# voidful/DeSTA2.5-Audio

Measured on AMD Instinct MI355X. Metric: train steps/sec (node) Whisper-v3+Llama3.1-8B Q-Former6L at 1/2/4/8 MI355X, higher is better.
Workload: dtype bf16

## Files before the change

desta2.5-audio_amd/csrc/gemm_bf16.hip:

```cpp
#include "common.h"
#include "desta_hip.h"
#include <math.h>

#ifndef GEMM_GROUP_M
#define GEMM_GROUP_M 8
#endif

namespace {

typedef __attribute__((ext_vector_type(4))) unsigned u32x4;
typedef __attribute__((ext_vector_type(2))) float f32x2;

constexpr int BM = 128, BN = 128, BK = 64;
constexpr int TILE_BYTES = BM * BK * 2;

struct GemmArgs {
    const bf16_t* A; const bf16_t* B; void* C;
    int M, N, K;
    long lda, ldb, ldc;
    long sA, sB, sC;
    const float* bias;
    const void* res; long ldr; long sR; int res_f32;
    int act;
    int out_f32;
// ... 381 lines not shown
        bf16x4_t v;
        asm volatile("ds_read_b64_tr_b16 %0, %1" : "=v"(v) : "v"((unsigned)(unsigned long)(img + off)) : "memory");
        o[4 * s2 + 0] = v[0]; o[4 * s2 + 1] = v[1]; o[4 * s2 + 2] = v[2]; o[4 * s2 + 3] = v[3];
    }
    return o;
}

template <bool TA, bool TB>
__global__ __launch_bounds__(256, 2) void gemm_bf16_nt_ring_kernel(GemmArgs p) {
    constexpr int NS = 4;
    __shared__ __attribute__((aligned(16))) char lds[NS * 2 * TILE_BYTES];

    const int tid = threadIdx.x, lane = tid & 63, wave = __builtin_amdgcn_readfirstlane(tid >> 6);
    const int wr = wave >> 1, wc = wave & 1;

    const int ntile = p.tilesM * p.tilesN;
    const int L = xcd_remap(blockIdx.x, ntile);
    constexpr int GROUP_M = 8;
    const int gspan = GROUP_M * p.tilesN;
    const int first_m = (L / gspan) * GROUP_M;
    const int gsz = min(p.tilesM - first_m, GROUP_M);
    const int tm = first_m + (L % gspan) % gsz;
    const int tn = (L % gspan) / gsz;
    const int brow = tm * BM, bcol = tn * BN;
    const int z = blockIdx.y;

    const bf16_t* A = p.A + (long)z * p.sA;
    const bf16_t* B = p.B + (long)z * p.sB;

    const bf16_t* srcA[4];
    const bf16_t* srcB[4];
#pragma unroll
    for (int i = 0; i < 4; ++i) {
        const int idx = i * 256 + tid;
        if (TA) {
            const int k = idx >> 4, c = (idx & 15) ^ tr_swz(k);
            srcA[i] = A + (long)k * p.lda + min(brow + c * 8, p.M - 8);
        } else {
            const int r = idx >> 3, c = (idx & 7) ^ (r & 7);
            srcA[i] = A + (long)min(brow + r, p.M - 1) * p.lda + c * 8;
        }
        if (TB) {
            const int k = idx >> 4, c = (idx & 15) ^ tr_swz(k);
            srcB[i] = B + (long)k * p.ldb + min(bcol + c * 8, p.N - 8);
        } else {
            const int r = idx >> 3, c = (idx & 7) ^ (r & 7);
            srcB[i] = B + (long)min(bcol + r, p.N - 1) * p.ldb + c * 8;
        }
    }
    const long stepA = TA ? (long)BK * p.lda : BK, stepB = TB ? (long)BK * p.ldb : BK;
    const int nk = p.K / BK;
    auto stage = [&](int kt) {
        const int kc = min(kt, nk - 1);
        char* la = lds + (kt & (NS - 1)) * 2 * TILE_BYTES;
        char* lb = la + TILE_BYTES;
#pragma unroll
        for (int i = 0; i < 4; ++i) {
            const int wbase = (i * 256 + wave * 64) * 16;
            glds16(srcA[i] + kc * stepA, la + wbase);
            glds16(srcB[i] + kc * stepB, lb + wbase);
        }
    };

    f32x4 acc[4][4];
#pragma unroll
    for (int i = 0; i < 4; ++i)
#pragma unroll
        for (int j = 0; j < 4; ++j) acc[i][j] = f32x4{0.f, 0.f, 0.f, 0.f};

    const int fr = lane & 15, fq = lane >> 4;
    int offA[4], offB[4];
#pragma unroll
    for (int i = 0; i < 4; ++i) {
        const int ra = wr * 64 + i * 16 + fr;
        const int rb = wc * 64 + i * 16 + fr;
        offA[i] = ra * 128 + ((fq ^ (ra & 7)) << 4);
        offB[i] = rb * 128 + ((fq ^ (rb & 7)) << 4);
    }
    auto rd_a = [&](int kt, int kk, int i) __attribute__((always_inline)) -> bf16x8 {
        const char* la = lds + (kt & (NS - 1)) * 2 * TILE_BYTES;
        if (TA) return frag_trans_raw(la, wr * 64 + i * 16, kk, fr, fq);
        return *(const bf16x8*)(la + (offA[i] ^ (kk << 6)));
    };
    auto rd_b = [&](int kt, int kk, int i) __attribute__((always_inline)) -> bf16x8 {
        const char* lb = lds + (kt & (NS - 1)) * 2 * TILE_BYTES + TILE_BYTES;
        if (TB) return frag_trans_raw(lb, wc * 64 + i * 16, kk, fr, fq);
        return *(const bf16x8*)(lb + (offB[i] ^ (kk << 6)));
    };
    auto fence = [&]() __attribute__((always_inline)) { if (TA || TB) __builtin_amdgcn_sched_barrier(0); };
    auto landed = [&](bf16x8 (&af)[4], bf16x8 (&bfr)[4]) __attribute__((always_inline)) {
        asm volatile("s_waitcnt lgkmcnt(0)" : "+v"(af[0]), "+v"(af[1]), "+v"(af[2]), "+v"(af[3]), "+v"(bfr[0]), "+v"(bfr[1]), "+v"(bfr[2]), "+v"(bfr[3]) :: "memory");
    };

    stage(0); stage(1); stage(2);
    asm volatile("s_waitcnt vmcnt(16)" ::: "memory");
    __builtin_amdgcn_s_barrier();
    bf16x8 a0[4], b0[4], a1[4], b1[4];
#pragma unroll
    for (int i = 0; i < 4; ++i) { a0[i] = rd_a(0, 0, i); b0[i] = rd_b(0, 0, i); }
    landed(a0, b0);
    for (int kt = 0; kt < nk; ++kt) {
        {
            const int kc = min(kt + 3, nk - 1);
            char* la = lds + ((kt + 3) & (NS - 1)) * 2 * TILE_BYTES;
            char* lb = la + TILE_BYTES;
#pragma unroll
            for (int i = 0; i < 4; ++i) {
                const int wbase = (i * 256 + wave * 64) * 16;
                acc[i][0] = __builtin_amdgcn_mfma_f32_16x16x32_bf16(b0[0], a0[i], acc[i][0], 0, 0, 0);
                glds16(srcA[i] + kc * stepA, la + wbase);
                fence();
                acc[i][1] = __builtin_amdgcn_mfma_f32_16x16x32_bf16(b0[1], a0[i], acc[i][1], 0, 0, 0);
                a1[i] = rd_a(kt, 1, i);
                fence();
                acc[i][2] = __builtin_amdgcn_mfma_f32_16x16x32_bf16(b0[2], a0[i], acc[i][2], 0, 0, 0);
                glds16(srcB[i] + kc * stepB, lb + wbase);
                fence();
                acc[i][3] = __builtin_amdgcn_mfma_f32_16x16x32_bf16(b0[3], a0[i], acc[i][3], 0, 0, 0);
                b1[i] = rd_b(kt, 1, i);
                fence();
            }
            if (!TA && !TB) {
#pragma unroll
                for (int i = 0; i < 8; ++i) {
                    __builtin_amdgcn_sched_group_barrier(0x008, 1, 0);
                    __builtin_amdgcn_sched_group_barrier(0x020, 1, 0);
                    __builtin_amdgcn_sched_group_barrier(0x008, 1, 0);
                    __builtin_amdgcn_sched_group_barrier(0x100, 1, 0);
                }
            }
        }
        __builtin_amdgcn_sched_barrier(0);
        landed(a1, b1);
        asm volatile("s_waitcnt vmcnt(16)" ::: "memory");
        __builtin_amdgcn_s_barrier();
#pragma unroll
        for (int i = 0; i < 4; ++i) {
            acc[i][0] = __builtin_amdgcn_mfma_f32_16x16x32_bf16(b1[0], a1[i], acc[i][0], 0, 0, 0);
            acc[i][1] = __builtin_amdgcn_mfma_f32_16x16x32_bf16(b1[1], a1[i], acc[i][1], 0, 0, 0);
            a0[i] = rd_a(kt + 1, 0, i);
            fence();
            acc[i][2] = __builtin_amdgcn_mfma_f32_16x16x32_bf16(b1[2], a1[i], acc[i][2], 0, 0, 0);
            acc[i][3] = __builtin_amdgcn_mfma_f32_16x16x32_bf16(b1[3], a1[i], acc[i][3], 0, 0, 0);
            b0[i] = rd_b(kt + 1, 0, i);
            fence();
        }
        if (!TA && !TB) {
#pragma unroll
            for (int i = 0; i < 8; ++i) {
                __builtin_amdgcn_sched_group_barrier(0x008, 2, 0);
                __builtin_amdgcn_sched_group_barrier(0x100, 1, 0);
            }
        }
        __builtin_amdgcn_sched_barrier(0);
        landed(a0, b0);
    }
    asm volatile("s_waitcnt vmcnt(0)" ::: "memory");

    if constexpr (!TA && !TB) {
        if (p.act == 2 || p.act == 3) {
            const int ncol0 = bcol + wc * 64;
            if (ncol0 < p.N) {
#pragma unroll
                for (int i = 0; i < 4; ++i) {
                    const int m = brow + wr * 64 + i * 16 + fr;
                    if (p.act == 2) epilogue_swiglu_fwd(p, z, min(m, p.M - 1), m < p.M, ncol0, fq, acc[i][0], acc[i][1], acc[i][2], acc[i][3]);
                    else epilogue_swiglu_bwd(p, z, min(m, p.M - 1), m < p.M, ncol0, fq, acc[i][0], acc[i][1], acc[i][2], acc[i][3]);
                }
            }
            return;
        }
    }
#pragma unroll
    for (int i = 0; i < 4; ++i) {
        const int m = brow + wr * 64 + i * 16 + fr;
        if (m >= p.M) continue;
#pragma unroll
        for (int j = 0; j < 4; ++j) {
            const int n0 = bcol + wc * 64 + j * 16 + fq * 4;
            if (n0 >= p.N) continue;
            epilogue4<true>(p, z, m, n0, acc[i][j]);
        }
    }
}


constexpr int HT = 128 * BK * 2;

struct K256Stream {
    const bf16_t* src[4][2];
    char* lds;
    int kt0, nk, n_ht, wave;
    bool tskip;
    __device__ __forceinline__ void init(const GemmArgs& p, char* lds_, int tid, int wave_, const bf16_t* A, const bf16_t* B,
                                         int brow, int bcol, int kt0_, int nk_, bool tskip_) {
        lds = lds_; wave = wave_; kt0 = kt0_; nk = nk_; n_ht = 4 * nk_; tskip = tskip_;
#pragma unroll
        for (int i = 0; i < 2; ++i) {
            const int idx = i * 512 + tid;
            const int r = idx >> 3, pc = idx & 7;
            const int c = pc ^ (r & 7);
#pragma unroll
            for (int s2 = 0; s2 < 2; ++s2) {
                const int arow = (r >> 6) * 128 + s2 * 64 + (r & 63);
                const int bcolr = (r >> 5) * 64 + s2 * 32 + (r & 31);
                src[s2][i] = A + (long)min(brow + arow, p.M - 1) * p.lda + c * 8;
                src[2 + s2][i] = B + (long)min(bcol + bcolr, p.N - 1) * p.ldb + c * 8;
            }
        }
    }
    __device__ __forceinline__ void stage(int j) {
        if (tskip && j >= n_ht) return;
        const int t = j >> 2, q = j & 3;
        const int kind = (q == 0) ? 0 : (q == 1) ? 2 : (q == 2) ? 3 : 1;
        const long koff = (long)(kt0 + min(t, nk - 1)) * BK;
        char* dst = lds + ((t & 1) * 4 + kind) * HT;
#pragma unroll
        for (int i = 0; i < 2; ++i)
            glds16(src[kind][i] + koff, dst + (i * 512 + wave * 64) * 16);
    }
    __device__ __forceinline__ void stage_steady(int j) {
        const int t = j >> 2, q = j & 3;
        const int kind = (q == 0) ? 0 : (q == 1) ? 2 : (q == 2) ? 3 : 1;
        const long koff = (long)(kt0 + t) * BK;
        char* dst = lds + ((t & 1) * 4 + kind) * HT;
#pragma unroll
        for (int i = 0; i < 2; ++i)
            glds16(src[kind][i] + koff, dst + (i * 512 + wave * 64) * 16);
    }
    __device__ __forceinline__ void wait_steady(int) { asm volatile("s_waitcnt vmcnt(8)" ::: "memory"); }
    __device__ __forceinline__ void tail_wait(int issued) {
        const int ov = tskip ? issued - n_ht : 0;
        if (ov <= 0) asm volatile("s_waitcnt vmcnt(8)" ::: "memory");
        else if (ov == 1) asm volatile("s_waitcnt vmcnt(6)" ::: "memory");
        else if (ov == 2) asm volatile("s_waitcnt vmcnt(4)" ::: "memory");
        else if (ov == 3) asm volatile("s_waitcnt vmcnt(2)" ::: "memory");
        else asm volatile("s_waitcnt vmcnt(0)" ::: "memory");
    }
};

template <bool STAGGER, class AtTail>
__device__ __forceinline__ void k256_loop_2phase(K256Stream& st, const int (&offA)[4], const int (&offB)[2], f32x4 (&acc)[8][4],
                                                 AtTail&& at_tail) {
    const int nk = st.nk, wave = st.wave;
    const char* lds = st.lds;
    bf16x8 a[4][2], b0[2][2], b1[2][2];
#define MFMA_SLOT(ACC_I0, ACC_J0, BF)                                                                        \
    __builtin_amdgcn_sched_barrier(0);                                                                       \
    __builtin_amdgcn_s_setprio(1);                                                                           \
    _Pragma("unroll") for (int kk = 0; kk < 2; ++kk)                                                         \
        _Pragma("unroll") for (int i = 0; i < 4; ++i)                                                        \
            _Pragma("unroll") for (int j = 0; j < 2; ++j)                                                    \
                acc[ACC_I0 + i][ACC_J0 + j] =                                                                \
                    __builtin_amdgcn_mfma_f32_16x16x32_bf16(BF[j][kk], a[i][kk], acc[ACC_I0 + i][ACC_J0 + j], 0, 0, 0); \
    __builtin_amdgcn_s_setprio(0);                                                                           \
    __builtin_amdgcn_sched_barrier(0);
#define KTILE_2PHASE(STAGE, WAIT)                                                                              \
    {                                                                                                          \
        _Pragma("unroll") for (int i = 0; i < 2; ++i)                                                          \
            _Pragma("unroll") for (int kk = 0; kk < 2; ++kk) {                                                 \
                b0[i][kk] = *(const bf16x8*)(B0 + (offB[i] ^ (kk << 6)));                                      \
                b1[i][kk] = *(const bf16x8*)(B1 + (offB[i] ^ (kk << 6)));                                      \
            }                                                                                                  \
        _Pragma("unroll") for (int i = 0; i < 4; ++i)                                                          \
            _Pragma("unroll") for (int kk = 0; kk < 2; ++kk) a[i][kk] = *(const bf16x8*)(A0 + (offA[i] ^ (kk << 6))); \
        st.STAGE(g + 7);                                                                                       \
        asm volatile("s_waitcnt lgkmcnt(0)" ::: "memory");                                                     \
        if (STAGGER) { st.WAIT(g + 8); __builtin_amdgcn_s_barrier(); }                                         \
        MFMA_SLOT(0, 0, b0)                                                                                    \
        MFMA_SLOT(0, 2, b1)                                                                                    \
        st.WAIT(g + 8); __builtin_amdgcn_s_barrier();                                                          \
        _Pragma("unroll") for (int i = 0; i < 4; ++i)                                                          \
            _Pragma("unroll") for (int kk = 0; kk < 2; ++kk) a[i][kk] = *(const bf16x8*)(A1 + (offA[i] ^ (kk << 6))); \
        st.STAGE(g + 8);                                                                                       \
        st.STAGE(g + 9);                                                                                       \
        st.STAGE(g + 10);                                                                                      \
        asm volatile("s_waitcnt lgkmcnt(0)" ::: "memory");                                                     \
        if (STAGGER) { st.WAIT(g + 11); __builtin_amdgcn_s_barrier(); }                                       \
        MFMA_SLOT(4, 2, b1)                                                                                    \
        MFMA_SLOT(4, 0, b0)                                                                                    \
        st.WAIT(g + 11); __builtin_amdgcn_s_barrier();                                                         \
    }
    if (STAGGER && wave >= 4) __builtin_amdgcn_s_barrier();
    const int nk_steady = max(nk - 2, 0);
    for (int t = 0; t < nk_steady; ++t) {
        const char* base = lds + (t & 1) * 4 * HT;
        const char* A0 = base, *A1 = base + HT, *B0 = base + 2 * HT, *B1 = base + 3 * HT;
        const int g = 4 * t;
        KTILE_2PHASE(stage_steady, wait_steady)
    }
    at_tail();
    for (int t = nk_steady; t < nk; ++t) {
        const char* base = lds + (t & 1) * 4 * HT;
        const char* A0 = base, *A1 = base + HT, *B0 = base + 2 * HT, *B1 = base + 3 * HT;
        const int g = 4 * t;
        KTILE_2PHASE(stage, tail_wait)
    }
    if (STAGGER && wave < 4) __builtin_amdgcn_s_barrier();
#undef KTILE_2PHASE
#undef MFMA_SLOT
}

constexpr int E256_DYN = -2, E256_SWIGLU_FWD = 32, E256_SWIGLU_BWD = 33, E256_F32_STREAM = 64;
template <int EPI>
__device__ __forceinline__ void k256_epilogue(const GemmArgs& p, int z, int brow, int bcol, int wm, int wn, int fr, int fq,
                                              const f32x4 (&acc)[8][4]) {
    if constexpr (EPI == E256_SWIGLU_FWD || EPI == E256_SWIGLU_BWD) {
        const int ncol0 = bcol + wn * 64;
        if (ncol0 < p.N) {
#pragma unroll
            for (int i = 0; i < 8; ++i) {
                const int m = brow + wm * 128 + i * 16 + fr;
                if (EPI == E256_SWIGLU_FWD) epilogue_swiglu_fwd(p, z, min(m, p.M - 1), m < p.M, ncol0, fq, acc[i][0], acc[i][1], acc[i][2], acc[i][3]);
                else epilogue_swiglu_bwd(p, z, min(m, p.M - 1), m < p.M, ncol0, fq, acc[i][0], acc[i][1], acc[i][2], acc[i][3]);
            }
        }
        return;
    }
#define DESTA_WIDE_TILE(MODE)                                                                                          \
        _Pragma("unroll") for (int i = 0; i < 8; ++i) {                                                                \
            const int m = brow + wm * 128 + i * 16 + fr;                                                               \
            const int mc = min(m, p.M - 1);                                                                            \
            _Pragma("unroll") for (int j = 0; j < 4; j += 2) {                                                         \
                const int ncol0 = bcol + wn * 64 + j * 16;                                                             \
                if (ncol0 >= p.N) continue;                                                          \
                epilogue_pair_bf16<MODE>(p, z, mc, m < p.M, ncol0, fq, acc[i][j], acc[i][j + 1]);    \
            }                                                                                                          \
        }
#define DESTA_F32_STREAM_TILE()                                                                                        \
        _Pragma("unroll") for (int i = 0; i < 8; ++i) {                                                                \
            const int m = brow + wm * 128 + i * 16 + fr;                                                               \
            if (m >= p.M) continue;                                                                                    \
            _Pragma("unroll") for (int j = 0; j < 4; ++j) {                                                            \
                const int n0 = bcol + wn * 64 + j * 16 + fq * 4;                                                       \
                if (n0 >= p.N) continue;                                                                               \
                epilogue4_f32_stream(p, z, m, n0, acc[i][j]);                                                          \
            }                                                                                                          \
        }
    if constexpr (EPI == E256_F32_STREAM) {
        DESTA_F32_STREAM_TILE()
    } else if constexpr (EPI >= 0) {
        DESTA_WIDE_TILE(EPI)
    } else {
        const bool pre_ok = !p.preact || (p.act == 0 && !p.res && (p.ldp & 7) == 0 && (p.sP & 7) == 0);
        const bool wide = !p.out_f32 && pre_ok && p.act <= 1 && !p.drop_thresh && (p.N % 32 == 0) && (p.ldc % 8 == 0);
        if (wide) {
            DESTA_WIDE_TILE(-1)
            return;
        }
#pragma unroll
        for (int i = 0; i < 8; ++i) {
            const int m = brow + wm * 128 + i * 16 + fr;
            if (m >= p.M) continue;
#pragma unroll
            for (int j = 0; j < 4; ++j) {
                const int n0 = bcol + wn * 64 + j * 16 + fq * 4;
                if (n0 >= p.N) continue;
                epilogue4(p, z, m, n0, acc[i][j]);
            }
        }
    }
#undef DESTA_F32_STREAM_TILE
#undef DESTA_WIDE_TILE
}

__device__ __forceinline__ void k256_store_slab(float* slab, int wm, int wn, int fr, int fq, const f32x4 (&acc)[8][4]) {
#pragma unroll
    for (int i = 0; i < 8; ++i)
#pragma unroll
        for (int j = 0; j < 4; ++j)
            *(f32x4*)(slab + (wm * 128 + i * 16 + fr) * 256 + wn * 64 + j * 16 + fq * 4) = acc[i][j];
}

template <bool STAGGER, int PHASES, int EPI = 0>
__global__ __launch_bounds__(512, 2) void gemm_bf16_nt_256_kernel(GemmArgs p) {
    __shared__ __attribute__((aligned(16))) char lds[2 * 4 * HT];

    const int tid = threadIdx.x, lane = tid & 63, wave = __builtin_amdgcn_readfirstlane(tid >> 6);
    const int wm = wave >> 2, wn = wave & 3;

    int L, slice = 0;
    if ((int)blockIdx.x < p.full_tiles) {
        L = xcd_remap(blockIdx.x, p.full_tiles);
    } else {
        const int j = blockIdx.x - p.full_tiles;
        L = p.full_tiles + j / p.split;
        slice = j % p.split;
    }
    constexpr int GROUP_M = GEMM_GROUP_M;
    const int gspan = GROUP_M * p.tilesN;
    const int first_m = (L / gspan) * GROUP_M;
    const int gsz = min(p.tilesM - first_m, GROUP_M);
    const int tm = first_m + (L % gspan) % gsz;
    const int tn = (L % gspan) / gsz;
    const int brow = tm * 256, bcol = tn * 256;
    const int z = blockIdx.y;
    const bf16_t* A = p.A + (long)z * p.sA;
    const bf16_t* B = p.B + (long)z * p.sB;

    const int nk_all = p.K / BK;
    const bool partial = (int)blockIdx.x >= p.full_tiles && p.split > 1;
    const int kt0 = partial ? (int)((long)nk_all * slice / p.split) : 0;
    const int kt1 = partial ? (int)((long)nk_all * (slice + 1) / p.split) : nk_all;
    const int nk = kt1 - kt0;
    K256Stream st;
    st.init(p, lds, tid, wave, A, B, brow, bcol, kt0, nk, PHASES == 2 && p.tail_skip != 0);

    f32x4 acc[8][4];
#pragma unroll
    for (int i = 0; i < 8; ++i)
#pragma unroll
        for (int j = 0; j < 4; ++j) acc[i][j] = f32x4{0.f, 0.f, 0.f, 0.f};

    const int fr = lane & 15, fq = lane >> 4;
    int offA[4], offB[2];
#pragma unroll
    for (int i = 0; i < 4; ++i) {
        const int r = wm * 64 + i * 16 + fr;
        offA[i] = r * 128 + ((fq ^ (r & 7)) << 4);
    }
#pragma unroll
    for (int i = 0; i < 2; ++i) {
        const int r = wn * 32 + i * 16 + fr;
        offB[i] = r * 128 + ((fq ^ (r & 7)) << 4);
    }

#pragma unroll
    for (int j = 0; j < 7; ++j) st.stage(j);
    if (PHASES == 4) asm volatile("s_waitcnt vmcnt(10)" ::: "memory");
    else st.tail_wait(7);
    __builtin_amdgcn_s_barrier();

    if constexpr (PHASES == 2) {
        k256_loop_2phase<STAGGER>(st, offA, offB, acc, [] {});
    } else {
        bf16x8 a[4][2], b0[2][2], b1[2][2];
#define SLOT_END()                                                                                                  \
    asm volatile("s_waitcnt vmcnt(10)" ::: "memory");                                                               \
    __builtin_amdgcn_s_barrier();
#define MFMA_SLOT(ACC_I0, ACC_J0, BF)                                                                        \
    __builtin_amdgcn_sched_barrier(0);                                                                       \
    __builtin_amdgcn_s_setprio(1);                                                                           \
    _Pragma("unroll") for (int kk = 0; kk < 2; ++kk)                                                         \
        _Pragma("unroll") for (int i = 0; i < 4; ++i)                                                        \
            _Pragma("unroll") for (int j = 0; j < 2; ++j)                                                    \
                acc[ACC_I0 + i][ACC_J0 + j] =                                                                \
                    __builtin_amdgcn_mfma_f32_16x16x32_bf16(BF[j][kk], a[i][kk], acc[ACC_I0 + i][ACC_J0 + j], 0, 0, 0); \
    __builtin_amdgcn_s_setprio(0);                                                                           \
    __builtin_amdgcn_sched_barrier(0);
        if (STAGGER && wave >= 4) __builtin_amdgcn_s_barrier();
        for (int t = 0; t < nk; ++t) {
            const char* base = lds + (t & 1) * 4 * HT;
            const char* A0 = base, *A1 = base + HT, *B0 = base + 2 * HT, *B1 = base + 3 * HT;
            const int g = 4 * t;
#pragma unroll
            for (int i = 0; i < 2; ++i)
#pragma unroll
                for (int kk = 0; kk < 2; ++kk) b0[i][kk] = *(const bf16x8*)(B0 + (offB[i] ^ (kk << 6)));
#pragma unroll
            for (int i = 0; i < 4; ++i)
#pragma unroll
                for (int kk = 0; kk < 2; ++kk) a[i][kk] = *(const bf16x8*)(A0 + (offA[i] ^ (kk << 6)));
            st.stage(g + 7);
            asm volatile("s_waitcnt lgkmcnt(0)" ::: "memory");
            if (STAGGER) { SLOT_END() }
            MFMA_SLOT(0, 0, b0)
            SLOT_END()
#pragma unroll
            for (int i = 0; i < 2; ++i)
#pragma unroll
                for (int kk = 0; kk < 2; ++kk) b1[i][kk] = *(const bf16x8*)(B1 + (offB[i] ^ (kk << 6)));
            st.stage(g + 8);
            asm volatile("s_waitcnt lgkmcnt(0)" ::: "memory");
            if (STAGGER) { SLOT_END() }
            MFMA_SLOT(0, 2, b1)
            SLOT_END()
#pragma unroll
            for (int i = 0; i < 4; ++i)
#pragma unroll
                for (int kk = 0; kk < 2; ++kk) a[i][kk] = *(const bf16x8*)(A1 + (offA[i] ^ (kk << 6)));
            st.stage(g + 9);
            asm volatile("s_waitcnt lgkmcnt(0)" ::: "memory");
            if (STAGGER) { SLOT_END() }
            MFMA_SLOT(4, 2, b1)
            SLOT_END()
            st.stage(g + 10);
            if (STAGGER) { SLOT_END() }
            MFMA_SLOT(4, 0, b0)
            SLOT_END()
        }
        if (STAGGER && wave < 4) __builtin_amdgcn_s_barrier();
#undef MFMA_SLOT
#undef SLOT_END
    }
    asm volatile("s_waitcnt vmcnt(0)" ::: "memory");

    if (partial) {
        float* slab = p.ws + ((long)z * (p.tilesM * p.tilesN - p.full_tiles) * p.split +
                              (long)(blockIdx.x - p.full_tiles)) * (256 * 256);
        k256_store_slab(slab, wm, wn, fr, fq, acc);
        if (!p.tickets) return;
        __shared__ int s_go;
        int* tk = p.tickets + 2 * ((long)z * (p.tilesM * p.tilesN - p.full_tiles) + (L - p.full_tiles));
        asm volatile("s_waitcnt vmcnt(0)" ::: "memory");
        __syncthreads();
        if (tid == 0) {
            __builtin_amdgcn_fence(__ATOMIC_RELEASE, "agent");
            asm volatile("s_waitcnt vmcnt(0)" ::: "memory");
            __hip_atomic_fetch_add(tk, 1, __ATOMIC_RELAXED, __HIP_MEMORY_SCOPE_AGENT);
            int spins = 0, ok = 1;
            while (__hip_atomic_load(tk, __ATOMIC_RELAXED, __HIP_MEMORY_SCOPE_AGENT) < p.split) {
                __builtin_amdgcn_s_sleep(2);
                if (++spins > (1 << 21)) { ok = 0; break; }
            }
            __builtin_amdgcn_fence(__ATOMIC_ACQUIRE, "agent");
            asm volatile("s_waitcnt vmcnt(0)" ::: "memory");
            s_go = ok;
        }
        __syncthreads();
        if (s_go) {
            const float* s0 = p.ws + ((long)z * (p.tilesM * p.tilesN - p.full_tiles) + (L - p.full_tiles)) * p.split * (256 * 256);
            const int r0 = 256 * slice / p.split, r1 = 256 * (slice + 1) / p.split;
            for (int idx = tid; idx < (r1 - r0) * 64; idx += 512) {
                const int ml = r0 + (idx >> 6), nl = (idx & 63) * 4;
                const float* q = s0 + ml * 256 + nl;
                f32x4 v = *(const f32x4*)q;
                for (int s2 = 1; s2 < p.split; ++s2) {
                    const f32x4 w = *(const f32x4*)(q + (long)s2 * (256 * 256));
                    v[0] += w[0]; v[1] += w[1]; v[2] += w[2]; v[3] += w[3];
                }
                const int m = brow + ml, n0 = bcol + nl;
                if (m < p.M && n0 < p.N) epilogue4<true>(p, z, m, n0, v);
            }
        }
        __syncthreads();
        if (tid == 0) {
            const int dpt = __hip_atomic_fetch_add(tk + 1, 1, __ATOMIC_RELAXED, __HIP_MEMORY_SCOPE_AGENT);
            if (dpt == p.split - 1) {
                __hip_atomic_store(tk, 0, __ATOMIC_RELAXED, __HIP_MEMORY_SCOPE_AGENT);
                __hip_atomic_store(tk + 1, 0, __ATOMIC_RELAXED, __HIP_MEMORY_SCOPE_AGENT);
            }
        }
        return;
    }
    if constexpr (EPI == 1) {
        const int ncol0 = bcol + wn * 64;
        if (ncol0 < p.N) {
#pragma unroll
            for (int i = 0; i < 8; ++i) {
                const int m = brow + wm * 128 + i * 16 + fr;
                if (p.act == 2) epilogue_swiglu_fwd(p, z, min(m, p.M - 1), m < p.M, ncol0, fq, acc[i][0], acc[i][1], acc[i][2], acc[i][3]);
                else epilogue_swiglu_bwd(p, z, min(m, p.M - 1), m < p.M, ncol0, fq, acc[i][0], acc[i][1], acc[i][2], acc[i][3]);
            }
        }
        return;
    }
    const bool pre_ok = !p.preact || (p.act == 0 && !p.res && (p.ldp & 7) == 0 && (p.sP & 7) == 0);
    const bool wide = !p.out_f32 && pre_ok && p.act <= 1 && !p.drop_thresh && (p.N % 32 == 0) && (p.ldc % 8 == 0);
    if (wide) {
#define DESTA_WIDE_TILE(MODE)                                                                                          \
        _Pragma("unroll") for (int i = 0; i < 8; ++i) {                                                                \
            const int m = brow + wm * 128 + i * 16 + fr;                                                               \
            const int mc = min(m, p.M - 1);                                                                            \
            _Pragma("unroll") for (int j = 0; j < 4; j += 2) {                                                         \
                const int ncol0 = bcol + wn * 64 + j * 16;                                                             \
                if (ncol0 >= p.N) continue;                                                          \
                epilogue_pair_bf16<MODE>(p, z, mc, m < p.M, ncol0, fq, acc[i][j], acc[i][j + 1]);    \
            }                                                                                                          \
        }
        const int mode = (p.bias ? 1 : 0) | (p.act == 1 ? 2 : 0) | (p.rope_cs ? 4 : 0) | (p.res ? 8 : 0) | (p.preact ? 16 : 0);
        if (mode == 0) { DESTA_WIDE_TILE(0) }
        else if (mode == 8) { DESTA_WIDE_TILE(8) }
        else if (mode == 4) { DESTA_WIDE_TILE(4) }
        else if (mode == 1) { DESTA_WIDE_TILE(1) }
        else if (mode == 3) { DESTA_WIDE_TILE(3) }
        else if (mode == 16) { DESTA_WIDE_TILE(16) }
        else { DESTA_WIDE_TILE(-1) }
#undef DESTA_WIDE_TILE
        return;
    }
    if (p.out_f32 && p.bias && p.res && p.res_f32 && !p.preact && p.act == 0 && !p.drop_thresh) {
#pragma unroll
        for (int i = 0; i < 8; ++i) {
            const int m = brow + wm * 128 + i * 16 + fr;
            if (m >= p.M) continue;
#pragma unroll
            for (int j = 0; j < 4; ++j) {
                const int n0 = bcol + wn * 64 + j * 16 + fq * 4;
                if (n0 >= p.N) continue;
                epilogue4_f32_stream(p, z, m, n0, acc[i][j]);
            }
        }
        return;
    }
#pragma unroll
    for (int i = 0; i < 8; ++i) {
        const int m = brow + wm * 128 + i * 16 + fr;
        if (m >= p.M) continue;
#pragma unroll
        for (int j = 0; j < 4; ++j) {
            const int n0 = bcol + wn * 64 + j * 16 + fq * 4;
            if (n0 >= p.N) continue;
            epilogue4(p, z, m, n0, acc[i][j]);
        }
    }
}

constexpr int P256_SLICES_FIRST = 1;
template <int EPI, bool TAIL>
__global__ __launch_bounds__(512, 2) void gemm_bf16_nt_256p_kernel(GemmArgs p, int* queue, int flags_) {
    static_assert(!TAIL || (EPI != E256_SWIGLU_FWD && EPI != E256_SWIGLU_BWD), "the SwiGLU epilogues need whole tiles");
    const int flags = TAIL ? flags_ : 0;
    __shared__ __attribute__((aligned(16))) char lds[2 * 4 * HT + 16];
    int* s_ticket = (int*)(lds + 2 * 4 * HT);
    const int tid = threadIdx.x, lane = tid & 63, wave = __builtin_amdgcn_readfirstlane(tid >> 6);
    const int wm = wave >> 2, wn = wave & 3;
    const int fr = lane & 15, fq = lane >> 4;
    constexpr int GROUP_M = GEMM_GROUP_M;
    const int nk_all = p.K / BK;

    const int xq = blockIdx.x & 7;
    const int F = p.full_tiles, q8 = F >> 3, r8 = F & 7;
    const int lo = (xq < r8) ? xq * (q8 + 1) : r8 * (q8 + 1) + (xq - r8) * q8;
    const int n_full = q8 + (xq < r8 ? 1 : 0);
    const int n_split_items = TAIL ? (p.tilesM * p.tilesN - F) * p.split : 0;
    const int n_slices = n_split_items > xq ? (n_split_items - xq + 7) >> 3 : 0;
    const int n_items = n_full + n_slices;
    const int s_lo = (flags & P256_SLICES_FIRST) ? 0 : n_full;
    const int w_lo = (flags & P256_SLICES_FIRST) ? n_slices : 0;
    int* counter = queue + xq;

    int brow, bcol, kt0, nk, slab;
    bool partial;
    auto geometry = [&](int tk) {
        int L, slice = 0;
        partial = tk >= s_lo && tk < s_lo + n_slices;
        if (!partial) {
            L = lo + tk - w_lo;
        } else {
            slab = xq + 8 * (tk - s_lo);
            L = F + slab / p.split;
            slice = slab % p.split;
        }
        const int gspan = GROUP_M * p.tilesN;
        const int first_m = (L / gspan) * GROUP_M;
        const int gsz = min(p.tilesM - first_m, GROUP_M);
        brow = (first_m + (L % gspan) % gsz) * 256;
        bcol = ((L % gspan) / gsz) * 256;
        kt0 = partial ? (int)((long)nk_all * slice / p.split) : 0;
        const int kt1 = partial ? (int)((long)nk_all * (slice + 1) / p.split) : nk_all;
        nk = kt1 - kt0;
    };
    auto draw = [&]() { return __hip_atomic_fetch_add(counter, 1, __ATOMIC_RELAXED, __HIP_MEMORY_SCOPE_AGENT); };

    int offA[4], offB[2];
#pragma unroll
    for (int i = 0; i < 4; ++i) {
        const int r = wm * 64 + i * 16 + fr;
        offA[i] = r * 128 + ((fq ^ (r & 7)) << 4);
    }
#pragma unroll
    for (int i = 0; i < 2; ++i) {
        const int r = wn * 32 + i * 16 + fr;
        offB[i] = r * 128 + ((fq ^ (r & 7)) << 4);
    }

    if (tid == 0) *s_ticket = draw();
    __syncthreads();
    int tk = *s_ticket;
    K256Stream st;
    if (tk < n_items) {
        geometry(tk);
        st.init(p, lds, tid, wave, p.A, p.B, brow, bcol, kt0, nk, p.tail_skip != 0);
#pragma unroll
        for (int j = 0; j < 7; ++j) st.stage(j);
    }
    f32x4 acc[8][4];
    while (tk < n_items) {
#pragma unroll
        for (int i = 0; i < 8; ++i)
#pragma unroll
            for (int j = 0; j < 4; ++j) acc[i][j] = f32x4{0.f, 0.f, 0.f, 0.f};
        st.tail_wait(7);
        __builtin_amdgcn_s_barrier();
        int nxt;
        k256_loop_2phase<true>(st, offA, offB, acc, [&] {
            const unsigned lane_mask = __builtin_amdgcn_readfirstlane(wave == 0 ? 1u : 0u);
            unsigned long saved;
            asm volatile("s_mov_b64 %1, exec\n\t"
                         "s_mov_b32 exec_lo, %3\n\t"
                         "s_mov_b32 exec_hi, 0\n\t"
                         "global_atomic_add %0, %2, %4, off sc0\n\t"
                         "s_mov_b64 exec, %1"
                         : "=&v"(nxt), "=&s"(saved) : "v"(counter), "s"(lane_mask), "v"(1) : "memory");
        });
        asm volatile("s_waitcnt vmcnt(0)" ::: "memory");
        if (tid == 0) *s_ticket = nxt;
        __syncthreads();
        const int cur_brow = brow, cur_bcol = bcol, cur_slab = slab;
        const bool cur_partial = partial;
        tk = *s_ticket;
        if (tk < n_items) {
            geometry(tk);
            st.init(p, lds, tid, wave, p.A, p.B, brow, bcol, kt0, nk, p.tail_skip != 0);
#pragma unroll
            for (int j = 0; j < 7; ++j) st.stage(j);
        }
        if constexpr (TAIL) {
            if (cur_partial) {
                k256_store_slab(p.ws + (long)cur_slab * (256 * 256), wm, wn, fr, fq, acc);
                continue;
            }
        }
        k256_epilogue<EPI>(p, 0, cur_brow, cur_bcol, wm, wn, fr, fq, acc);
    }
    asm volatile("s_waitcnt vmcnt(0)" ::: "memory");
    __syncthreads();
    if (tid == 0) {
        const int dpt = __hip_atomic_fetch_add(queue + 8, 1, __ATOMIC_RELAXED, __HIP_MEMORY_SCOPE_AGENT);
        if (dpt == (int)gridDim.x - 1) {
#pragma unroll
            for (int k = 0; k < 9; ++k) __hip_atomic_store(queue + k, 0, __ATOMIC_RELAXED, __HIP_MEMORY_SCOPE_AGENT);
        }
    }
}

__global__ __launch_bounds__(256) void gemm_splitk_fixup_kernel(GemmArgs p) {
    const int rem = p.tilesM * p.tilesN - p.full_tiles;
    const int ti = blockIdx.x / 64, part = blockIdx.x % 64;
    const int z = blockIdx.y;
    const int L = p.full_tiles + ti;
    constexpr int GROUP_M = GEMM_GROUP_M;
    const int gspan = GROUP_M * p.tilesN;
    const int first_m = (L / gspan) * GROUP_M;
    const int gsz = min(p.tilesM - first_m, GROUP_M);
    const int tm = first_m + (L % gspan) % gsz;
    const int tn = (L % gspan) / gsz;
    const int ml = part * 4 + (threadIdx.x >> 6), nl = (threadIdx.x & 63) * 4;
    const float* slab = p.ws + ((long)z * rem + ti) * p.split * (256 * 256) + ml * 256 + nl;
    f32x4 acc = *(const f32x4*)slab;
    for (int s2 = 1; s2 < p.split; ++s2) {
        const f32x4 v = *(const f32x4*)(slab + (long)s2 * (256 * 256));
        acc[0] += v[0]; acc[1] += v[1]; acc[2] += v[2]; acc[3] += v[3];
    }
    const int m = tm * 256 + ml, n0 = tn * 256 + nl;
    if (m < p.M && n0 < p.N) epilogue4<true>(p, z, m, n0, acc);
}

template <int COLS, int U, bool W8>
struct SkinnyStage {
    bf16x8 w0[U][COLS / 16], w1[U][COLS / 16], x0[U], x1[U];
};
template <int COLS, int U>
struct SkinnyStage<COLS, U, true> {
    u32x4 wq[U][COLS / 16];
    bf16x8 x0[U], x1[U];
};

__device__ __forceinline__ void e4m3x16_to_bf16(const u32x4& q, bf16x8& lo, bf16x8& hi) {
    union { unsigned u[8]; bf16x8 v[2]; } o;
#pragma unroll
    for (int i = 0; i < 4; ++i) {
        const f32x2 a = __builtin_amdgcn_cvt_pk_f32_fp8((int)q[i], false), b = __builtin_amdgcn_cvt_pk_f32_fp8((int)q[i], true);
        o.u[2 * i] = __builtin_amdgcn_perm(__float_as_uint(a[1]), __float_as_uint(a[0]), 0x07060302u);
        o.u[2 * i + 1] = __builtin_amdgcn_perm(__float_as_uint(b[1]), __float_as_uint(b[0]), 0x07060302u);
    }
    lo = o.v[0]; hi = o.v[1];
}

constexpr int SKINNY_XS_BYTES = 8 * 4096 * 2;
struct SkinnyCursor { int tile, grp; };
#ifndef SKINNY_W8_U
#define SKINNY_W8_U 2
#endif

__device__ __forceinline__ u16x4 swiglu4_bf16(const f32x4& gs, const f32x4& us, float alpha) {
    u16x4 o;
#pragma unroll
    for (int e = 0; e < 4; ++e) {
        const float gt = bf2f(f2bf(gs[e] * alpha)), uu = bf2f(f2bf(us[e] * alpha));
        o[e] = f2bf(bf2f(f2bf(gt / (1.0f + __expf(-gt)))) * uu);
    }
    return o;
}

__device__ __forceinline__ void rms_rows_to_lds(const GemmArgs& p, const bf16_t* A, char* xs, int wave, int lane) {
    for (int m = wave; m < p.M; m += 8) {
        const bf16_t* xr = A + (long)m * p.lda;
        float q = 0.f;
#pragma unroll 4
        for (int c = lane * 8; c < p.K; c += 512) {
            const u16x8 v = *(const u16x8*)(xr + c);
#pragma unroll
            for (int e = 0; e < 8; ++e) { const float f = bf2f(v[e]); q += f * f; }
        }
        const float rstd = rsqrtf(wave_sum(q) / (float)p.K + p.rms_eps);
#pragma unroll 2
        for (int c = lane * 8; c < p.K; c += 512) {
            const u16x8 v = *(const u16x8*)(xr + c);
            const float4 w0 = *(const float4*)(p.rms_w + c), w1 = *(const float4*)(p.rms_w + c + 4);
            const float wv[8] = {w0.x, w0.y, w0.z, w0.w, w1.x, w1.y, w1.z, w1.w};
            u16x8 o;
#pragma unroll
            for (int e = 0; e < 8; ++e) o[e] = f2bf(wv[e] * bf2f(f2bf(bf2f(v[e]) * rstd)));
            *(u16x8*)(xs + m * (p.K * 2) + (((c >> 3) ^ m) << 4)) = o;
        }
    }
    __syncthreads();
}

template <int COLS, int U, bool SWIGLU, bool RMS, bool W8 = false>
__global__ __launch_bounds__(512, (COLS == 16 && (U == 2 || W8)) ? 2 : 1) void gemm_bf16_nt_skinny_kernel(GemmArgs p, int ntiles) {
    static_assert(!SWIGLU || COLS == 16, "SwiGLU pairing uses one 16-row weight tile");
    constexpr int T = COLS / 16;
    constexpr int RED_BYTES = 8 * T * 64 * 16;
    __shared__ __attribute__((aligned(16))) char smem[2 * RED_BYTES + (RMS ? SKINNY_XS_BYTES : 0)];
    const char* xs = smem + 2 * RED_BYTES;
    const int lane = threadIdx.x & 63, wave = threadIdx.x >> 6, z = blockIdx.y;
    const int r = lane & 15, g = lane >> 4;
    const bool mok = r < p.M;
    const bf16_t* Bz = p.B + (long)z * p.sB + g * 16;
    const char* Bq = (const char*)p.B + (long)z * p.sB + g * 16;
    const bf16_t* ap = p.A + (long)z * p.sA + (long)(mok ? r : 0) * p.lda + g * 16;
    const int nchunks = p.K >> 6;
    constexpr int STEP = 8 * U;
    const int gpt = (nchunks + STEP - 1) / STEP;
    const int my_tiles = ((int)blockIdx.x < ntiles) ? (ntiles - (int)blockIdx.x + (int)gridDim.x - 1) / (int)gridDim.x : 0;
    const int G = my_tiles * gpt;
    const int rowb = p.K * 2, rr = mok ? r : 0;
    const char* xrow = xs + rr * rowb;
    f32x4 acc[T];
#pragma unroll
    for (int t = 0; t < T; ++t) acc[t] = f32x4{0.f, 0.f, 0.f, 0.f};
    SkinnyStage<COLS, U, W8> sa, sb;
    SkinnyCursor lc = {(int)blockIdx.x, 0}, mc = {(int)blockIdx.x, 0};
    int parity = 0;

    auto advance = [&](SkinnyCursor& c) { if (++c.grp == gpt) { c.grp = 0; c.tile += (int)gridDim.x; } };
#define SK_LOAD(S)                                                                          \
    {                                                                                       \
        const int n0 = lc.tile * (SWIGLU ? 8 : COLS), c0 = wave + lc.grp * STEP;            \
        const bf16_t* bp[T];                                                                \
        const char* bq[T];                                                                  \
        _Pragma("unroll") for (int t = 0; t < T; ++t) {       \
            const int wrow = SWIGLU ? (r < 8 ? min(n0 + r, p.N - 1) : p.N + min(n0 + r - 8, p.N - 1)) \
                                    : min(n0 + t * 16 + r, p.N - 1);                        \
            bp[t] = Bz + (long)wrow * p.ldb;                                                \
            bq[t] = Bq + (long)wrow * p.ldb;                                                \
        }                                                                                   \
        _Pragma("unroll") for (int u = 0; u < U; ++u) {                                     \
            const int cc = c0 + 8 * u;                                                      \
            if (cc < nchunks) {                                                             \
                _Pragma("unroll") for (int t = 0; t < T; ++t) {                             \
                    if constexpr (W8) {                                                     \
                        S.wq[u][t] = *(const u32x4*)(bq[t] + (long)cc * 64);                \
                    } else {                                                                \
                        S.w0[u][t] = *(const bf16x8*)(bp[t] + (long)cc * 64);               \
                        S.w1[u][t] = *(const bf16x8*)(bp[t] + (long)cc * 64 + 8);           \
                    }                                                                       \
                }                                                                           \
                if (!RMS) {                                                                 \
                    S.x0[u] = *(const bf16x8*)(ap + (long)cc * 64);                         \
                    S.x1[u] = *(const bf16x8*)(ap + (long)cc * 64 + 8);                     \
                }                                                                           \
            }                                                                               \
        }                                                                                   \
        advance(lc);                                                                        \
    }
#define SK_MMA(S)                                                                           \
    {                                                                                       \
        const int c0 = wave + mc.grp * STEP;                                                \
        _Pragma("unroll") for (int u = 0; u < U; ++u) {                                     \
            if (c0 + 8 * u < nchunks) {                                                     \
                const bf16x8 zero = {};                                                     \
                if (RMS) {                                                                  \
                    const int slot = (c0 + 8 * u) * 8 + g * 2;                              \
                    S.x0[u] = *(const bf16x8*)(xrow + ((slot ^ rr) << 4));                  \
                    S.x1[u] = *(const bf16x8*)(xrow + (((slot + 1) ^ rr) << 4));            \
                }                                                                           \
                const bf16x8 a0 = mok ? S.x0[u] : zero, a1 = mok ? S.x1[u] : zero;          \
                _Pragma("unroll") for (int t = 0; t < T; ++t) {                             \
                    if constexpr (W8) {                                                     \
                        bf16x8 w0, w1;                                                      \
                        e4m3x16_to_bf16(S.wq[u][t], w0, w1);                                \
                        acc[t] = __builtin_amdgcn_mfma_f32_16x16x32_bf16(w0, a0, acc[t], 0, 0, 0); \
                        acc[t] = __builtin_amdgcn_mfma_f32_16x16x32_bf16(w1, a1, acc[t], 0, 0, 0); \
                    } else {                                                                \
                        acc[t] = __builtin_amdgcn_mfma_f32_16x16x32_bf16(S.w0[u][t], a0, acc[t], 0, 0, 0); \
                        acc[t] = __builtin_amdgcn_mfma_f32_16x16x32_bf16(S.w1[u][t], a1, acc[t], 0, 0, 0); \
                    }                                                                       \
                }                                                                           \
            }                                                                               \
        }                                                                                   \
        if (mc.grp == gpt - 1) finish_tile(mc.tile);                                        \
        advance(mc);                                                                        \
    }
    auto finish_tile = [&](int tile) {
        f32x4 (*red)[T][64] = (f32x4 (*)[T][64])(smem + parity * RED_BYTES);
        parity ^= 1;
#pragma unroll
        for (int t = 0; t < T; ++t) { red[wave][t][lane] = acc[t]; acc[t] = f32x4{0.f, 0.f, 0.f, 0.f}; }
        __syncthreads();
        if (wave < T) {
            f32x4 sum = red[0][wave][lane];
#pragma unroll
            for (int w = 1; w < 8; ++w) sum += red[w][wave][lane];
            const int n0 = tile * (SWIGLU ? 8 : COLS);
            if constexpr (W8) {
                const int n = SWIGLU ? n0 + (g & 1) * 4 : n0 + wave * 16 + g * 4;
                if (n < p.N) {
                    const float4 s = *(const float4*)(p.b_scale + (SWIGLU && g >= 2 ? p.N : 0) + n);
                    sum[0] *= s.x; sum[1] *= s.y; sum[2] *= s.z; sum[3] *= s.w;
                }
            }
            if (SWIGLU) {
                f32x4 up;
#pragma unroll
                for (int e = 0; e < 4; ++e) up[e] = __shfl(sum[e], (lane + 32) & 63, 64);
                const u16x4 o = swiglu4_bf16(sum, up, p.alpha);
                const int n = n0 + g * 4;
                if (mok && g < 2 && n < p.N) *(u16x4*)((bf16_t*)p.C + (long)z * p.sC + (long)r * p.ldc + n) = o;
            } else {
                const int n = n0 + wave * 16 + g * 4;
                if (mok && n < p.N) epilogue4(p, z, r, n, sum);
            }
        }
    };

    if (G > 0) SK_LOAD(sa)
    if (RMS) rms_rows_to_lds(p, p.A + (long)z * p.sA, smem + 2 * RED_BYTES, wave, lane);
    for (int gi = 0; gi < G; gi += 2) {
        if (gi + 1 < G) SK_LOAD(sb)
        SK_MMA(sa)
        if (gi + 2 < G) SK_LOAD(sa)
        if (gi + 1 < G) SK_MMA(sb)
    }
#undef SK_LOAD
#undef SK_MMA
}

template <int MF, bool W8>
struct WideStage {
    bf16x8 w0[4], w1[4], x0[MF], x1[MF];
};
template <int MF>
struct WideStage<MF, true> {
    u32x4 wq[4];
    bf16x8 x0[MF], x1[MF];
};

struct WideCursor { int item, grp, tile, slice; };
template <bool SWIGLU>
struct WideWalk {
    int N, ntiles, ks, cps, nchunks;
    int ntot, gpt, G;
    __device__ WideWalk(int N_, int ntiles_, int ks_, int cps_, int nchunks_) : N(N_), ntiles(ntiles_), ks(ks_), cps(cps_), nchunks(nchunks_) {
        ntot = SWIGLU ? 2 * N : N;
        gpt = (cps + 7) >> 3;
        const int items = ntiles * ks;
        const int my_items = ((int)blockIdx.x < items) ? (items - (int)blockIdx.x + (int)gridDim.x - 1) / (int)gridDim.x : 0;
        G = my_items * gpt;
    }
    __device__ WideCursor first() const { return {(int)blockIdx.x, 0, (int)blockIdx.x % ntiles, (int)blockIdx.x / ntiles}; }
    __device__ void advance(WideCursor& c) const {
        if (++c.grp == gpt) { c.grp = 0; c.item += (int)gridDim.x; c.tile = c.item % ntiles; c.slice = c.item / ntiles; }
    }
    __device__ int chunk(const WideCursor& c, int wave) const { return c.slice * cps + wave + c.grp * 8; }
    __device__ int chunk_end(const WideCursor& c) const { return min((c.slice + 1) * cps, nchunks); }
    __device__ int wrow(int tile, int t, int q, bool& ok) const {
        if (SWIGLU) {
            const int n = tile * 32 + (t & 1) * 16 + q;
            ok = n < N;
            return (t >= 2 ? N : 0) + min(n, N - 1);
        }
        const int n = tile * 64 + t * 16 + q;
        ok = n < N;
        return min(n, N - 1);
    }
};

template <bool ON>
struct RowScale {
    const float* s;
    __device__ f32x4 operator()(f32x4 sum, int row) const {
        if constexpr (ON) {
            const float4 v = *(const float4*)(s + row);
            sum[0] *= v.x; sum[1] *= v.y; sum[2] *= v.z; sum[3] *= v.w;
        }
        return sum;
    }
};

template <int MF, bool SWIGLU, class Scale>
struct WideFinish {
    const GemmArgs& p; const WideWalk<SWIGLU>& wk; f32x4 (*const& red)[4 * MF][64]; f32x4 (&acc)[4][MF];
    const int& lane; const int& wave; const int& r; const int& g; float* const& part; Scale scaled;
    __device__ f32x4 reduced(int t, int f) const {
        f32x4 sum = red[0][t * MF + f][lane];
#pragma unroll
        for (int w = 1; w < 8; ++w) sum += red[w][t * MF + f][lane];
        return sum;
    }
    __device__ void operator()(int tile, int slice) const {
        constexpr int T = 4;
#pragma unroll
        for (int t = 0; t < T; ++t)
#pragma unroll
            for (int f = 0; f < MF; ++f) { red[wave][t * MF + f][lane] = acc[t][f]; acc[t][f] = f32x4{0.f, 0.f, 0.f, 0.f}; }
        __syncthreads();
        if (wk.ks > 1) {
            for (int u = wave; u < T * MF; u += 8) {
                const int t = u / MF, f = u % MF, m = f * 16 + r;
                bool ok;
                const int row = wk.wrow(tile, t, g * 4, ok);
                if (ok && m < p.M) *(f32x4*)(part + ((long)slice * p.M + m) * wk.ntot + row) = reduced(t, f);
            }
        } else if (SWIGLU) {
// ... 615 lines not shown
```

Measured before the change: 6.683.

## Add batched, prefetching epilogues for residual, bias and f32-stream 256-tile GEMM outputs

Adds specialized epilogue paths for full-width 256x256 tiles. Residual reads (bf16 and f32) are double-buffered in batches so loads overlap with the arithmetic and stores. Bias vectors are loaded once per thread instead of per element, and output packing uses permlane swaps for wide stores. The aim is to cut the latency-bound per-element loads in the epilogue, at the cost of extra registers, an explicit waitcnt before the residual loads, and more code paths to keep correct.

```diff
diff --git a/desta2.5-audio_amd/csrc/gemm_bf16.hip b/desta2.5-audio_amd/csrc/gemm_bf16.hip
--- a/desta2.5-audio_amd/csrc/gemm_bf16.hip
+++ b/desta2.5-audio_amd/csrc/gemm_bf16.hip
@@ -707,9 +707,119 @@
 }
 
 constexpr int E256_DYN = -2, E256_SWIGLU_FWD = 32, E256_SWIGLU_BWD = 33, E256_F32_STREAM = 64;
-template <int EPI>
+
+__device__ __forceinline__ void k256_dma_booked_off() { __builtin_amdgcn_s_waitcnt(0xC07F); }
+constexpr int K256_STREAM_DEPTH = 4;
+constexpr int K256_RES_DEPTH = 4;
+
+__device__ __forceinline__ void k256_f32_stream_batched(const GemmArgs& p, int z, int brow, int bcol, int wm, int wn, int fr, int fq,
+                                                        const f32x4 (&acc)[8][4]) {
+    constexpr int D = K256_STREAM_DEPTH, NB = 32 / D;
+    const int m0 = brow + wm * 128 + fr, n00 = bcol + wn * 64 + fq * 4;
+    float4 bias[4];
+#pragma unroll
+    for (int j = 0; j < 4; ++j) bias[j] = *(const float4*)(p.bias + n00 + j * 16);
+    float4 r[2][D];
+    auto fetch = [&](int b) {
+#pragma unroll
+        for (int s = 0; s < D; ++s) {
+            const int i = (b * D + s) >> 2, j = (b * D + s) & 3;
+            r[b & 1][s] = *(const float4*)((const float*)p.res + (long)z * p.sR + (long)min(m0 + i * 16, p.M - 1) * p.ldr + n00 + j * 16);
+        }
+    };
+    k256_dma_booked_off();
+    fetch(0);
+#pragma unroll
+    for (int b = 0; b < NB; ++b) {
+        if (b + 1 < NB) fetch(b + 1);
+#pragma unroll
+        for (int s = 0; s < D; ++s) {
+            const int i = (b * D + s) >> 2, j = (b * D + s) & 3;
+            const f32x4& a = acc[i][j];
+            const float4 bb = bias[j], rr = r[b & 1][s];
+            const float4 o = make_float4((a[0] * p.alpha + bb.x) + rr.x, (a[1] * p.alpha + bb.y) + rr.y, (a[2] * p.alpha + bb.z) + rr.z, (a[3] * p.alpha + bb.w) + rr.w);
+            if (m0 + i * 16 < p.M) *(float4*)((float*)p.C + (long)z * p.sC + (long)(m0 + i * 16) * p.ldc + n00 + j * 16) = o;
+        }
+    }
+}
+
+__device__ __forceinline__ void k256_residual_batched(const GemmArgs& p, int z, int brow, int bcol, int wm, int wn, int fr, int fq,
+                                                      const f32x4 (&acc)[8][4]) {
+    constexpr int D = K256_RES_DEPTH, NB = 16 / D;
+    const int m0 = brow + wm * 128 + fr, col0 = bcol + wn * 64 + (fq & 1) * 16 + (fq >> 1) * 8;
+    u16x8 r[2][D];
+    auto fetch = [&](int b) {
+#pragma unroll
+        for (int s = 0; s < D; ++s) {
+            const int i = (b * D + s) >> 1, jp = (b * D + s) & 1;
+            r[b & 1][s] = *(const u16x8*)((const bf16_t*)p.res + (long)z * p.sR + (long)min(m0 + i * 16, p.M - 1) * p.ldr + col0 + jp * 32);
+        }
+    };
+    k256_dma_booked_off();
+    fetch(0);
+#pragma unroll
+    for (int b = 0; b < NB; ++b) {
+        if (b + 1 < NB) fetch(b + 1);
+#pragma unroll
+        for (int s = 0; s < D; ++s) {
+            const int i = (b * D + s) >> 1, jp = (b * D + s) & 1;
+            const f32x4 &a0 = acc[i][2 * jp], &a1 = acc[i][2 * jp + 1];
+            float w[8];
+#pragma unroll
+            for (int e = 0; e < 4; ++e) {
+                const auto sw = __builtin_amdgcn_permlane16_swap(__float_as_uint(a0[e] * p.alpha), __float_as_uint(a1[e] * p.alpha), false, false);
+                w[e] = __uint_as_float(sw[0]);
+                w[4 + e] = __uint_as_float(sw[1]);
+            }
+            u16x8 o;
+#pragma unroll
+            for (int e = 0; e < 8; ++e) o[e] = f2bf(w[e] + bf2f(r[b & 1][s][e]));
+            if (m0 + i * 16 < p.M) *(u16x8*)((bf16_t*)p.C + (long)z * p.sC + (long)(m0 + i * 16) * p.ldc + col0 + jp * 32) = o;
+        }
+    }
+}
+
+template <bool GELU>
+__device__ __forceinline__ void k256_bias_once(const GemmArgs& p, int z, int brow, int bcol, int wm, int wn, int fr, int fq,
+                                               const f32x4 (&acc)[8][4]) {
+    const int m0 = brow + wm * 128 + fr, ncol = bcol + wn * 64;
+    float4 bias[4];
+#pragma unroll
+    for (int j = 0; j < 4; ++j) bias[j] = *(const float4*)(p.bias + ncol + j * 16 + fq * 4);
+#pragma unroll
+    for (int i = 0; i < 8; ++i) {
+#pragma unroll
+        for (int jp = 0; jp < 2; ++jp) {
+            unsigned pk[2][2];
+#pragma unroll
+            for (int t = 0; t < 2; ++t) {
+                const f32x4& a = acc[i][2 * jp + t];
+                const float4 b = bias[2 * jp + t];
+                float v[4];
+#pragma unroll
+                for (int e = 0; e < 4; ++e) v[e] = a[e] * p.alpha;
+                v[0] += b.x; v[1] += b.y; v[2] += b.z; v[3] += b.w;
+                if (GELU) gelu4_bf16(v);
+                pk[t][0] = pk2(v[0], v[1]);
+                pk[t][1] = pk2(v[2], v[3]);
+            }
+            const uint4 o = pair_swap_pk(pk[0][0], pk[0][1], pk[1][0], pk[1][1]);
+            if (m0 + i * 16 < p.M) *(uint4*)((bf16_t*)p.C + (long)z * p.sC + (long)(m0 + i * 16) * p.ldc + ncol + jp * 32 + (fq & 1) * 16 + (fq >> 1) * 8) = o;
+        }
+    }
+}
+
+template <int EPI, bool BATCHED = true>
 __device__ __forceinline__ void k256_epilogue(const GemmArgs& p, int z, int brow, int bcol, int wm, int wn, int fr, int fq,
                                               const f32x4 (&acc)[8][4]) {
+    const bool cols_inside = BATCHED && bcol + 256 <= p.N;
+    if constexpr (EPI == E256_F32_STREAM) {
+        if (cols_inside) { k256_f32_stream_batched(p, z, brow, bcol, wm, wn, fr, fq, acc); return; }
+    } else if constexpr (EPI == 8) {
+        if (cols_inside && !p.res_f32 && (p.ldr & 7) == 0 && (p.sR & 7) == 0) { k256_residual_batched(p, z, brow, bcol, wm, wn, fr, fq, acc); return; }
+    } else if constexpr (EPI == 1 || EPI == 3) {
+        if (cols_inside) { k256_bias_once<EPI == 3>(p, z, brow, bcol, wm, wn, fr, fq, acc); return; }
+    }
     if constexpr (EPI == E256_SWIGLU_FWD || EPI == E256_SWIGLU_BWD) {
         const int ncol0 = bcol + wn * 64;
         if (ncol0 < p.N) {
@@ -948,6 +1058,7 @@
         }
         return;
     }
+    const bool cols_inside = bcol + 256 <= p.N;
     if constexpr (EPI == 1) {
         const int ncol0 = bcol + wn * 64;
         if (ncol0 < p.N) {
@@ -975,16 +1086,26 @@
         }
         const int mode = (p.bias ? 1 : 0) | (p.act == 1 ? 2 : 0) | (p.rope_cs ? 4 : 0) | (p.res ? 8 : 0) | (p.preact ? 16 : 0);
         if (mode == 0) { DESTA_WIDE_TILE(0) }
-        else if (mode == 8) { DESTA_WIDE_TILE(8) }
+        else if (mode == 8) {
+            if (cols_inside && !p.res_f32 && (p.ldr & 7) == 0 && (p.sR & 7) == 0) k256_residual_batched(p, z, brow, bcol, wm, wn, fr, fq, acc);
+            else { DESTA_WIDE_TILE(8) }
+        }
         else if (mode == 4) { DESTA_WIDE_TILE(4) }
-        else if (mode == 1) { DESTA_WIDE_TILE(1) }
-        else if (mode == 3) { DESTA_WIDE_TILE(3) }
+        else if (mode == 1) {
+            if (cols_inside) k256_bias_once<false>(p, z, brow, bcol, wm, wn, fr, fq, acc);
+            else { DESTA_WIDE_TILE(1) }
+        }
+        else if (mode == 3) {
+            if (cols_inside) k256_bias_once<true>(p, z, brow, bcol, wm, wn, fr, fq, acc);
+            else { DESTA_WIDE_TILE(3) }
+        }
         else if (mode == 16) { DESTA_WIDE_TILE(16) }
         else { DESTA_WIDE_TILE(-1) }
 #undef DESTA_WIDE_TILE
         return;
     }
     if (p.out_f32 && p.bias && p.res && p.res_f32 && !p.preact && p.act == 0 && !p.drop_thresh) {
+        if (cols_inside) { k256_f32_stream_batched(p, z, brow, bcol, wm, wn, fr, fq, acc); return; }
 #pragma unroll
         for (int i = 0; i < 8; ++i) {
             const int m = brow + wm * 128 + i * 16 + fr;
@@ -1117,7 +1238,7 @@
                 continue;
             }
         }
-        k256_epilogue<EPI>(p, 0, cur_brow, cur_bcol, wm, wn, fr, fq, acc);
+        k256_epilogue<EPI, !(TAIL && EPI == E256_F32_STREAM)>(p, 0, cur_brow, cur_bcol, wm, wn, fr, fq, acc);
     }
     asm volatile("s_waitcnt vmcnt(0)" ::: "memory");
     __syncthreads();
```

New measurement: 6.683 (median of 2 runs). No clear change (+0.0%).
